# AU-Master-Thesis/magics

Hardware: AMD Instinct MI355X
Metric: GBP iterations/sec (whole node), N robots x K horizon (higher is better)
Workload: dtype f64

## Files before the change

include/mgx.h:

```cpp
#ifndef MGX_H
#define MGX_H

#include <stdint.h>

#ifdef __cplusplus
extern "C" {
#endif

#define MGX_DOFS 4

#define MGX_OK 0
#define MGX_ERR_INVALID (-1)
#define MGX_ERR_NO_DEVICE (-2)
#define MGX_ERR_HIP (-3)
#define MGX_ERR_STATE (-4)
#define MGX_ERR_NOMEM (-5)

#define MGX_FACTOR_DYNAMIC 1u
#define MGX_FACTOR_INTERROBOT 2u
#define MGX_FACTOR_OBSTACLE 4u
#define MGX_FACTOR_TRACKING 8u

#define MGX_STEP_INTERNAL 1u
#define MGX_STEP_EXTERNAL 2u
// ... 76 lines not shown
#define MGX_SWEEP_FORM_SHARDED 3
int mgx_last_sweep(mgx_world *w, int32_t *variant, int32_t *ir_mode, int32_t *form, int32_t *resident_capacity);
#define MGX_SEARCH_NONE -1
#define MGX_SEARCH_TWO_PASS_PAIRS 0
#define MGX_SEARCH_TWO_PASS_GRID 1
#define MGX_SEARCH_ROWS_PAIRS_4 2
#define MGX_SEARCH_ROWS_PAIRS_2 3
#define MGX_SEARCH_ROWS_GRID_16 4
#define MGX_SEARCH_ROWS_GRID_32 5
int mgx_last_search(mgx_world *w, int32_t *kernel, int32_t *row_cap, int32_t *n_launches, int32_t *n_changed, uint8_t *changed,
                    uint32_t capacity);

int mgx_flush(mgx_world *w);
int mgx_set_linger(mgx_world *w, int32_t microseconds );
int mgx_linger_stats(mgx_world *w, uint64_t *launches, uint64_t *posts, uint64_t *reruns, uint64_t *ended_by_device);
int mgx_set_resident_launches(mgx_world *w, int32_t enabled);
int mgx_is_thawing(mgx_world *w, int32_t *thawing);

#define MGX_HINT_NEXT_STARTS_EXTERNAL 1u
int mgx_sweep(mgx_world *w, int32_t robot, uint32_t external_phases, uint32_t internal_phases,
              uint32_t n_internal, uint32_t hints);

int mgx_internal_factor_iteration(mgx_world *w, int32_t robot);
int mgx_internal_variable_iteration(mgx_world *w, int32_t robot);
int mgx_external_factor_iteration(mgx_world *w, int32_t robot);
int mgx_external_variable_iteration(mgx_world *w, int32_t robot);

int mgx_change_prior(mgx_world *w, int32_t robot, uint32_t var_ix, const double mean[4]);
int mgx_change_priors(mgx_world *w, uint32_t n, const int32_t *robots, const uint32_t *var_ix,
                      const double *means);
// ... 300 lines not shown
```

include/mgx.hpp:

```cpp
#pragma once

#include <array>
#include <cstdint>
#include <limits>
#include <memory>
#include <optional>
#include <stdexcept>
#include <string>
#include <utility>
#include <vector>

#include "mgx.h"

namespace mgx {

struct Error : std::runtime_error {
    int code;
    Error(int c, const std::string &what) : std::runtime_error(what), code(c) {}
};
inline int check(int rc) {
    if (rc < 0) throw Error(rc, mgx_last_error());
    return rc;
}

// ... 115 lines not shown
        check(mgx_ir_connect(w_, owner.id(), other.id(), numbers.next_value));
        numbers.next_value += K_ - 1;
    }
    void tick(const std::vector<int32_t> &robots, const std::vector<double> &waypoints_xy, const std::vector<double> &time_scale,
              const std::vector<uint8_t> &what, double max_speed, double delta_t, const std::vector<uint8_t> &steps) {
        check(mgx_tick(w_, (uint32_t)robots.size(), robots.data(), waypoints_xy.data(), time_scale.data(), what.data(), max_speed,
                       delta_t, steps.data(), (uint32_t)steps.size()));
    }
    uint32_t last_launch_count() {
        uint32_t n = 0;
        check(mgx_last_launch_count(w_, &n));
        return n;
    }
    void flush() { check(mgx_flush(w_)); }
    void set_linger(int32_t microseconds) { check(mgx_set_linger(w_, microseconds)); }
    void change_factor_enabled(uint32_t kind_mask) { check(mgx_set_enabled(w_, kind_mask)); }
    void update_inter_robot_safety_distance_multiplier(double multiplier) { check(mgx_set_safety_multiplier(w_, multiplier)); }
    std::pair<uint32_t, uint32_t> update_topology(const std::vector<std::array<float, 3>> &translations, float comms_radius,
                                                  RobotNumberGenerator &numbers) {
        uint32_t stats[2] = {0, 0};
        check(mgx_update_topology(w_, translations[0].data(), comms_radius, MGX_NEIGHBOURS_AUTO, &numbers.next_value, stats));
        return {stats[0], stats[1]};
    }
    void iterate_gbp_v2(const std::vector<GbpScheduleAtIteration> &sched) {
        std::vector<uint8_t> steps(sched.size());
        for (size_t i = 0; i < sched.size(); i++) steps[i] = (uint8_t)((sched[i].internal ? MGX_STEP_INTERNAL : 0) | (sched[i].external ? MGX_STEP_EXTERNAL : 0));
        check(mgx_iterate(w_, steps.data(), (uint32_t)steps.size()));
    }
    struct Batch {
        mgx_world *w;
// ... 235 lines not shown
```

magics_amd/csrc/mgx_resident.h:

```cpp
#pragma once
#include <algorithm>
#include <cstddef>
#include <cstdint>
#include <vector>

namespace mgx {

#ifndef __HIPCC__
constexpr uint32_t PH_INT_FACTOR = 4u, PH_INT_VARIABLE = 8u;
constexpr int MAX_SEGS = 32;
#endif
static_assert((PH_INT_FACTOR | PH_INT_VARIABLE) == 12u && MAX_SEGS == 32, "the phases and the plan's size as mgx_dev.h has them");

struct Launch { uint32_t ext; int n_int; uint32_t hints; };
inline uint32_t int_phases(const Launch &l) { return l.n_int ? (PH_INT_FACTOR | PH_INT_VARIABLE) : 0; }

inline int fill_segments(const std::vector<Launch> &plan, size_t from, uint8_t *ext, uint8_t *n_int) {
    const int n = (int)std::min<size_t>((size_t)MAX_SEGS, plan.size() - std::min(from, plan.size()));
    for (int k = 0; k < MAX_SEGS; k++) {
        ext[k] = k < n && plan[from + (size_t)k].ext ? 1 : 0;
        n_int[k] = k < n ? (uint8_t)plan[from + (size_t)k].n_int : 0;
    }
    return n;
}
// ... 3 lines not shown
    unsigned long long flag_base = 0;
    Standing after_launch(int n) const { return {(cur + n) & 1, flag_base + (unsigned long long)n}; }
    Standing after_post(int n) const { return after_launch(n - 1); }
};

struct Backoff {
    int left = 0, len = 0;
    void declined(int segments) {
        len = std::min(std::max(2 * len, 64), 32768);
        left = len + segments;
    }
    void external_iteration() { if (left > 0) left--; }
    void went_ahead() { len = 0; }
};

struct RidingUpdates {
    const double *dev = nullptr;
    const double *host = nullptr;
    int slot = -1;
    double max_speed = 0.0, delta_t = 0.0;
    bool any() const { return dev || host; }
    bool postable() const { return !dev || host; }
};

}
```

magics_amd/csrc/mgx_world_abi.inc:

```
extern "C" {

const char *mgx_last_error(void) { return g_err.c_str(); }
int mgx_set_error_(int code, const char *text) {
    g_err = text ? text : "";
    return code;
}

int mgx_world_create(const mgx_params *params, mgx_world **out) {
    if (!params || !out) return fail(MGX_ERR_INVALID, "null argument");
    if (!(params->sigma_dynamics > 0) || !(params->sigma_interrobot > 0) || !(params->sigma_obstacle > 0) ||
        !(params->sigma_tracking > 0) || !(params->safety_multiplier > 0))
        return fail(MGX_ERR_INVALID, "sigmas and safety multiplier must be positive");
    if (!device_ok()) return fail(MGX_ERR_NO_DEVICE, "no usable HIP device (this library has no CPU path)");
    mgx_world *w = new (std::nothrow) mgx_world();
    if (!w) return fail(MGX_ERR_NOMEM, "out of memory");
    w->p = *params;
    w->trk_ever_on = (params->enable_mask & 8u) != 0;
    *out = w;
    return MGX_OK;
}

int mgx_world_destroy(mgx_world *w) {
    if (!w) return MGX_OK;
    w->batch.steps.clear();
// ... 32 lines not shown
    MGX_ENTER(w);
    if (!w) return fail(MGX_ERR_INVALID, "null world");
    return MGX_OK;
}
int mgx_set_linger(mgx_world *w, int32_t microseconds) {
    MGX_ENTER(w);
    if (!w) return fail(MGX_ERR_INVALID, "null world");
    w->res.set_linger(microseconds);
    return MGX_OK;
}
int mgx_linger_stats(mgx_world *w, uint64_t *launches, uint64_t *posts, uint64_t *reruns, uint64_t *ended_by_device) {
    MGX_ENTER_SCHEDULE(w);
    if (!w) return fail(MGX_ERR_INVALID, "null world");
    const ResidentLaunches::Linger &lg = w->res.linger;
    if (launches) *launches = lg.launches;
    if (posts) *posts = lg.posts + (lg.un.active ? 1u : 0u);
    if (reruns) *reruns = lg.reruns;
    if (ended_by_device) *ended_by_device = lg.ended_by_device;
    return MGX_OK;
}

int mgx_world_set_sdf(mgx_world *w, const uint8_t *rgb, uint32_t width, uint32_t height, double world_w, double world_h) {
    MGX_ENTER(w);
    if (!w || !rgb || !width || !height || !(world_w > 0) || !(world_h > 0)) return fail(MGX_ERR_INVALID, "bad sdf arguments");
    w->sdf_red.resize((size_t)width * height);
    for (size_t i = 0; i < w->sdf_red.size(); i++) w->sdf_red[i] = rgb[3 * i];
    w->sdf_w = width; w->sdf_h = height; w->world_w = world_w; w->world_h = world_h;
    w->dirty = w->relayout = true;
    return MGX_OK;
}

int mgx_world_set_environment(mgx_world *w, const mgx_env_desc *env) {
    MGX_ENTER(w);
// ... 346 lines not shown
```

magics_amd/csrc/mgx_world_launch.inc:

```
static int direct_exchange(mgx_world *w);
static int rccl_exchange(mgx_world *w);
static int sweep(mgx_world *w, int32_t robot, uint32_t ext_mask, uint32_t int_mask, int n_int, uint32_t hints = 0);
static void log_launch(mgx_world *w, int robot, uint32_t ext_mask, uint32_t int_mask, int n_int);

static void log_plan(mgx_world *w, const std::vector<Launch> &plan, size_t from = 0, size_t n = ~(size_t)0) {
    for (size_t k = from; k < plan.size() && k - from < n; k++) log_launch(w, -1, plan[k].ext, int_phases(plan[k]), plan[k].n_int);
}
static int run_segments(mgx_world *w, const std::vector<Launch> &plan, size_t from, const RidingUpdates &upd) {
    for (size_t k = from; k < plan.size(); k++) {
        const bool rides = k == from && upd.dev;
        if (rides) { w->d.upd = upd.dev; w->d.upd_max_speed = upd.max_speed; w->d.upd_delta_t = upd.delta_t; }
        int rc = sweep(w, -1, plan[k].ext, int_phases(plan[k]), plan[k].n_int, plan[k].hints);
        w->d.upd = nullptr;
        if (rides && upd.slot >= 0) {
            const hipError_t e = w->stage.release(upd.slot, w->stream);
            if (rc == MGX_OK && e != hipSuccess) rc = fail(MGX_ERR_HIP, "event record: %s", hipGetErrorString(e));
        }
        if (rc != MGX_OK) return rc;
    }
    return MGX_OK;
}
template <class F>
static int spin_until(F done) {
    const double t0 = StageTimer::now();
// ... 130 lines not shown
        if (w->thaw_kinds && (thawing || writes_snap)) HIP_TRY(launch_thaw_done(w->d, w->dev_of[(size_t)robot], 1, writes_snap ? 1 : 0, w->stream));
        log_launch(w, robot, 0, int_mask, n_int);
    }
    return MGX_OK;
}


struct ResidentKnobs {
    static long long positive(const char *name, long long dflt) { const char *e = getenv(name); const long long v = e ? atoll(e) : dflt; return v > 0 ? v : dflt; }
    static bool persistent() { static const bool v = [] { const char *e = getenv("MGX_PERSISTENT"); return !(e && e[0] == '0'); }(); return v; }
    static long long timeout_ticks() { static const long long v = positive("MGX_RESIDENT_TIMEOUT_MS", 2000) * 100000ll; return v; }
    static bool census() { static const bool v = [] { const char *e = getenv("MGX_RESIDENT_CENSUS"); return !(e && e[0] == '0'); }(); return v; }
    static long long census_ticks() { static const long long v = positive("MGX_RESIDENT_CENSUS_US", 200) * 100ll; return v; }
    static long long census_ticks_sharded() { static const long long v = positive("MGX_RESIDENT_CENSUS_SHARDED_US", 20000) * 100ll; return v; }
    static bool cooperative() { static const bool v = [] { const char *e = getenv("MGX_COOPERATIVE"); return e && e[0] == '1'; }(); return v; }
    static long long linger_ticks() {
        const char *off = getenv("MGX_LINGER"), *us = getenv("MGX_LINGER_US");
        const long long v = off && off[0] == '0' ? 0 : us ? atoll(us) : 300;
        return (v > 0 ? std::min<long long>(v, 1000000) : 0) * 100ll;
    }
};
static bool resident_enabled() { return ResidentKnobs::persistent(); }
static int ensure_resident_tables(mgx_world *w) {
    hipStream_t s = w->stream;
    const size_t R = (size_t)w->d.R_local;
    if (!w->res.sweep_abort_buf.p) {
        std::vector<unsigned long long> z(1, 0ull);
        HIP_TRY(w->res.sweep_abort_buf.upload(z, s));
        HIP_TRY(hipStreamSynchronize(s));
    }
// ... 79 lines not shown
enum ResidentFit { FITS, UNFIT_NOW, UNFIT_LDS, UNFIT_CAPACITY };
static ResidentFit resident_fits(mgx_world *w, bool sharded) {
    const DevWorld &d = w->d;
    if (!(d.ir_max_edges > 0 && !w->conns.empty() && !w->thaw_kinds && !w->ir_thaw_active && w->n_keyless == 0 && w->res.mode != ResidentLaunches::DECLINE))
        return UNFIT_NOW;
    if (sweep_lds_bytes(w->K, d.ir_max_edges, true) > sweep_resident_lds_max()) return UNFIT_LDS;
    return d.R_local + 1 > w->res.capacity_for(d, sharded) ? UNFIT_CAPACITY : FITS;
}

static int run_resident(mgx_world *w, const std::vector<Launch> &plan);
static long long linger_ticks(mgx_world *w) {
    ResidentLaunches::Linger &lg = w->res.linger;
    if (lg.ticks < 0) lg.ticks = ResidentKnobs::linger_ticks();
    return lg.ticks;
}
static double *linger_upd_slot(mgx_world *w, unsigned long long number) {
    ResidentLaunches::Linger &lg = w->res.linger;
    return reinterpret_cast<double *>(reinterpret_cast<char *>(lg.box()) + sizeof(LingerBox)) + (size_t)(number & 1ull) * lg.upd_stride;
}
static int ensure_linger_box(mgx_world *w) {
    ResidentLaunches::Linger &lg = w->res.linger;
    const size_t stride = ((size_t)4 * (size_t)std::max(w->d.R_local, 1) + 7) & ~(size_t)7;
    if (!lg.go.p) {
        std::vector<unsigned long long> z(1, 0ull);
        HIP_TRY(lg.go.upload(z, w->stream));
        HIP_TRY(hipStreamSynchronize(w->stream));
    }
    if (lg.box() && lg.upd_stride >= stride) return MGX_OK;
    const size_t grown = (stride + stride / 2 + 7) & ~(size_t)7;
    HIP_TRY(lg.box_mem.alloc(sizeof(LingerBox) + 2 * grown * sizeof(double)));
// ... 7 lines not shown
template <class F>
static int linger_wait(mgx_world *w, F pred, const char *what) {
    ResidentLaunches::Linger &lg = w->res.linger;
    const int r = spin_until([&] {
        if (pred()) return 1;
        const unsigned long long c = __atomic_load_n(&lg.box()->closed, __ATOMIC_ACQUIRE);
        return (c & 1ull) && (c >> 1) >= lg.seq0 ? 2 : 0;
    });
    if (r < 0) return fail(MGX_ERR_STATE, "lingering launch %llu: no answer from the device while waiting for %s (the stream does not advance)", lg.seq0, what);
    return r - 1;
}
static void linger_confirm(mgx_world *w) {
    ResidentLaunches::Linger &lg = w->res.linger;
    log_plan(w, lg.un.plan);
    lg.un.active = false;
    lg.posts++;
    lg.taken_in_launch++;
}
static int run_schedule(mgx_world *w, const std::vector<Launch> &plan, const RidingUpdates &upd, StageTimer *lap = nullptr) {
    const RidingUpdates outer = w->res.riding;
    w->res.riding = upd;
    const int resident = run_resident(w, plan);
    w->res.riding = outer;
    if (lap) lap->lap("resident launch enqueued");
    if (resident == 0) return run_segments(w, plan, 0, upd);
    const hipError_t e = upd.slot >= 0 ? w->stage.release(upd.slot, w->stream) : hipSuccess;
    if (resident < 0) return resident;
    return e == hipSuccess ? MGX_OK : fail(MGX_ERR_HIP, "event record: %s", hipGetErrorString(e));
}
static int linger_settle(mgx_world *w, bool nested = false) {
    ResidentLaunches::Linger &lg = w->res.linger;
    const uint32_t count_before = w->last_sweep_launches;
    const unsigned long long c = __atomic_load_n(&lg.box()->closed, __ATOMIC_ACQUIRE);
    lg.open = false;
    int rc = MGX_OK;
    if (lg.un.active && (c >> 1) >= lg.un.number) {
        linger_confirm(w);
    } else if (lg.un.active) {
        Submitted un = std::move(lg.un);
        lg.un = Submitted{};
        lg.reruns++;
        un.take_back(w);
        RidingUpdates upd;
        if (un.upd.any()) {
            const size_t bytes = 4 * (size_t)w->d.R_local * sizeof(double);
            void *hp = nullptr, *dp = nullptr;
            HIP_TRY(w->stage.acquire(bytes, &hp, &upd.slot));
            memcpy(hp, un.upd.host, bytes);
            HIP_TRY(hipHostGetDevicePointer(&dp, hp, 0));
            upd.dev = (const double *)dp;
            upd.host = (const double *)hp;
            upd.max_speed = un.upd.max_speed;
            upd.delta_t = un.upd.delta_t;
        }
        rc = run_schedule(w, un.plan, upd);
    }
    if (nested) w->last_sweep_launches = count_before;
    if (lg.taken_in_launch == 0) lg.useless++;
    else lg.useless = 0;
    return rc;
}
static int linger_close(mgx_world *w) {
    ResidentLaunches::Linger &lg = w->res.linger;
    if (!lg.open) return MGX_OK;
    const int rc = confirm_held(w);
    if (rc != MGX_OK || !lg.open) return rc;
    StageTimer clock("linger");
    __atomic_store_n(&lg.box()->close_req, lg.seq0, __ATOMIC_RELEASE);
    const int r = linger_wait(w, [] { return false; }, "the launch to end");
    if (r < 0) return r;
    clock.lap("closed");
    return linger_settle(w);
}
static bool linger_plan_fits(const std::vector<Launch> &plan) {
    if (plan.empty() || plan.size() > (size_t)MAX_SEGS || plan[0].ext) return false;
    for (const Launch &l : plan)
        if (l.n_int > 255) return false;
    return true;
}
static int linger_prepare_post(mgx_world *w, const std::vector<Launch> &plan) {
    ResidentLaunches &rl = w->res;
    ResidentLaunches::Linger &lg = rl.linger;
    if (!lg.open) return 0;
    {
        const uint32_t count_before = w->last_sweep_launches;
        const int rc = confirm_held(w);
        w->last_sweep_launches = count_before;
        if (rc != MGX_OK) return rc;
        if (!lg.open) return 0;
    }
    const bool fits = linger_plan_fits(plan) && !w->dirty && !w->conns_dirty && !w->flags_dirty && !w->thaw_kinds && !w->ir_thaw_active &&
                      w->n_keyless == 0 && rl.mode == ResidentLaunches::ON && (w->p.enable_mask & 2u) && rl.backoff.left == 0;
    if (!fits) {
        const int rc = linger_close(w);
        return rc != MGX_OK ? rc : 0;
    }
    int r = 0;
    if (lg.un.active) {
        const unsigned long long n = lg.un.number;
        r = linger_wait(w, [&] { return __atomic_load_n(&lg.box()->taken, __ATOMIC_ACQUIRE) >= n; }, "the last post to be taken");
        if (r == 0) linger_confirm(w);
    }
    if (r < 0) return r;
    if (r == 1) {
        lg.ended_by_device++;
        const int rc = linger_settle(w, true);
        return rc != MGX_OK ? rc : 0;
// ... 7 lines not shown
    LingerPlan &lp = lg.box()->plan[P & 1ull];
    lp.n = (uint32_t)plan.size();
    lp.has_upd = upd.any() ? 1u : 0u;
    uint8_t ext[MAX_SEGS], n_int[MAX_SEGS];
    fill_segments(plan, 0, ext, n_int);
    memcpy(lp.ext, ext, sizeof ext);
    memcpy(lp.n_int, n_int, sizeof n_int);
    lp.upd_max_speed = upd.max_speed;
    lp.upd_delta_t = upd.delta_t;
    lp.number = P;
    Submitted &un = lg.un;
    un.active = true;
    un.number = P;
    un.plan = plan;
    un.before = standing(w);
    un.upd = RidingUpdates{};
    if (upd.any()) {
        double *slot = linger_upd_slot(w, P);
        if (upd.host != slot) memcpy(slot, upd.host, 4 * (size_t)w->d.R_local * sizeof(double));
        un.upd.host = slot;
        un.upd.max_speed = upd.max_speed;
        un.upd.delta_t = upd.delta_t;
    }
    __atomic_store_n(&lg.box()->posted, P, __ATOMIC_RELEASE);
    stand_at(w, un.before.after_post((int)plan.size()));
    w->stale_kinds |= ~w->p.enable_mask & 15u;
    w->last_sweep_launches++;
    w->last_sweep = lg.ran;
    w->last_sweep_form = MGX_SWEEP_FORM_POSTED;
}
// ... 129 lines not shown
```

magics_amd/csrc/mgx_world_schedule.inc:

```
extern "C" {
static int submit_batch(mgx_world *w) {
    std::vector<uint8_t> st;
    st.swap(w->batch.steps);
    if (st.empty()) return MGX_OK;
    const int rc = iterate_now(w, st.data(), (uint32_t)st.size());
    w->batch.submissions++;
    w->batch.launches += w->last_sweep_launches;
    return rc;
}

int mgx_batch_begin(mgx_world *w) {
    if (!w) return fail(MGX_ERR_INVALID, "null world");
    if (w->batch.open) return fail(MGX_ERR_STATE, "a batch is open already");
    w->batch.open = true;
    w->batch.schedules = w->batch.submissions = w->batch.launches = 0;
    return MGX_OK;
}
int mgx_batch_end(mgx_world *w, uint32_t *n_schedules, uint32_t *n_launches) {
    if (!w) return fail(MGX_ERR_INVALID, "null world");
    if (!w->batch.open) return fail(MGX_ERR_STATE, "no batch is open");
    w->batch.open = false;
    const int rc = submit_batch(w);
    if (n_schedules) *n_schedules = w->batch.schedules;
    if (n_launches) *n_launches = w->batch.launches;
    return rc;
}

int mgx_iterate(mgx_world *w, const uint8_t *steps, uint32_t n) {
    if (!w || (!steps && n)) return fail(MGX_ERR_INVALID, "null argument");
    for (uint32_t i = 0; i < n; i++)
        if (steps[i] & ~(MGX_STEP_INTERNAL | MGX_STEP_EXTERNAL)) return fail(MGX_ERR_INVALID, "bad step %u", i);
    if (!w->batch.open) return iterate_now(w, steps, n);
    if (w->robots.empty()) return fail(MGX_ERR_STATE, "world has no robots");
    int rc0 = check_device_error(w);
    if (rc0 != MGX_OK) return rc0;
    mgx_world::Batch &b = w->batch;
    if (!b.steps.empty()) {
        std::vector<uint8_t> both(b.steps);
        both.insert(both.end(), steps, steps + n);
        if (plan_launches(both.data(), (uint32_t)both.size()).size() > (size_t)MAX_SEGS) {
            const int rc = submit_batch(w);
            if (rc != MGX_OK) return rc;
        }
    }
    b.steps.insert(b.steps.end(), steps, steps + n);
    b.schedules++;
    return MGX_OK;
}

static int iterate_now(mgx_world *w, const uint8_t *steps, uint32_t n) {
    const std::vector<Launch> plan = plan_launches(steps, n);
    const int rcc = confirm_held(w);
    if (rcc != MGX_OK) return rcc;
    w->last_sweep_launches = 0;
    w->last_sweep = SweepRan{};
    w->last_sweep_form = -1;
    w->res.schedule_issued();
    return run_schedule(w, plan, RidingUpdates{});
}

int mgx_internal_factor_iteration(mgx_world *w, int32_t robot) {
    MGX_ENTER(w);
    return w ? sweep(w, robot, 0, PH_INT_FACTOR, 1) : fail(MGX_ERR_INVALID, "null world");
}
int mgx_internal_variable_iteration(mgx_world *w, int32_t robot) {
    MGX_ENTER(w);
// ... 533 lines not shown
```

magics_amd/csrc/mgx_world_types.h:

```cpp
#pragma once
#include <hip/hip_runtime.h>

#include <algorithm>
#include <cmath>
#include <cstdarg>
#include <cstdio>
#include <cstdlib>
#include <dlfcn.h>
#include <cstring>
#include <map>
#include <memory>
#include <string>
#include <utility>
#include <vector>

#include "../../include/mgx.h"
#include "gbp_math.h"
#include "mgx_dev.h"
#include "mgx_grid.h"
#include "mgx_search.h"
#include "mgx_plan_pool.h"
#include "mgx_resident.h"

namespace mgx {
// ... 378 lines not shown
    void release() { if (p) (void)hipHostFree(p); p = nullptr; }
    hipError_t alloc(size_t bytes) {
        release();
        const hipError_t e = hipHostMalloc(&p, bytes, hipHostMallocMapped);
        if (e == hipSuccess) memset(p, 0, bytes);
        return e;
    }
};

struct Submitted {
    bool active = false;
    unsigned long long number = 0;
    std::vector<Launch> plan;
    Standing before;
    bool partial = false;
    RidingUpdates upd;
    void take_back(mgx_world *w);
};

struct ResidentLaunches {
    DevBuf<unsigned long long> sweep_flag_buf, sweep_abort_buf, census_buf, decision_buf;
    DevBuf<unsigned char> xrec_buf;
    MappedBlock decision_mem;
    unsigned long long *decision_host() const { return (unsigned long long *)decision_mem.p; }
    DevBuf<int32_t> peer_ptr_dev, peer_ptr_dev_b;
    size_t peer_idx_off = 0;
    std::vector<int32_t> peer_fill;
    bool peers_valid = false;
    unsigned long long flag_base = 0;
    unsigned long long launch_seq = 0;
// ... 12 lines not shown
        long long ticks = -1;
        MappedBlock box_mem;
        LingerBox *box() const { return (LingerBox *)box_mem.p; }
        size_t upd_stride = 0;
        DevBuf<unsigned long long> go;
        DevBuf<unsigned char> dev;
        size_t dev_stride = 0;
        bool open = false, hold = false;
        unsigned long long seq0 = 0;
        SweepRan ran;
        uint32_t taken_in_launch = 0;
        int useless = 0;
        uint32_t streak = 0;
        Submitted un;
        uint64_t launches = 0, posts = 0, reruns = 0, ended_by_device = 0;
    } linger;
    void arrays_rebuilt() {
        peers_valid = false;
        sweep_flag_buf.n = 0;
        flag_base = 0;
        cap = cap_sharded = -1;
    }
    void robots_appended() {
        peers_valid = false;
        sweep_flag_buf.n = 0;
        flag_base = 0;
    }
    void lds_footprint_changed() { cap = cap_sharded = -1; }
    void peers_rebuilt(bool built, size_t R, DevWorld &d) {
        if (built) {
// ... 70 lines not shown
    DevBuf<IrEdgeRec> ir_rec_b;
    DevBuf<int32_t> in_ptr_dev, in_ptr_dev_b, in_mid_dev;
    DevBuf<IrSlotRec> slot_recs, slot_recs_b;
    std::vector<int32_t> dev_in_ptr;
    DevBuf<int32_t> trk_record, path_ptr, iter_factor, ir_var_ptr, ir_var_mid;
    DevBuf<uint32_t> epoch0, epoch1;
    DevBuf<float> trk_last_pos, path_xy;
    DevBuf<uint8_t> ir_gate, antenna, idle, sdf;
    DevBuf<double> radius_dev;
    StageRing stage;
    unsigned long long *sweep_err_host = nullptr;
    struct Batch {
        bool open = false;
        std::vector<uint8_t> steps;
        uint32_t schedules = 0, submissions = 0, launches = 0;
    } batch;
    ResidentLaunches res;
    int sticky_rc = 0;
    struct ConnHot {
        int32_t owner, other, node_first, node_last;
        uint64_t first_number;
        int32_t dev_q;
        uint8_t has_fresh;
    };
    std::vector<ConnHot> conn_hot;
    ConnIndex cidx;
    struct Cum { std::vector<uint64_t> nIv, nEv, nEf, on_ir; } cum;
    bool conns_unsettled = false;
    std::vector<uint8_t> scratch_dead;
    std::vector<int32_t> scratch_dead_list;
// ... 239 lines not shown
```

magics_amd/hostlib.py:

```python
import ctypes as C
import os

_HERE = os.path.dirname(os.path.abspath(__file__))
LIB_PATH = os.path.join(_HERE, "lib", "libmgx.so")
FMA_LIB_PATH = os.path.join(_HERE, "lib", "libmgx_fma.so")

SCHEDULE_CENTERED = 0
SCHEDULE_SOON_AS_POSSIBLE = 1
SCHEDULE_LATE_AS_POSSIBLE = 2
SCHEDULE_INTERLEAVE_EVENLY = 3
SCHEDULE_HALF_BEGINNING_HALF_END = 4

STEP_INTERNAL = 1
STEP_EXTERNAL = 2
NEIGHBOURS_AUTO, NEIGHBOURS_PAIRS, NEIGHBOURS_GRID = 0, 1, 2
GLOBAL_PATH_RESET_TRACKING, GLOBAL_PATH_ROUTE, GLOBAL_PATH_ACTIVATE = 1, 2, 4
RESIDENT_NONE, RESIDENT_RAN, RESIDENT_DECLINED = 0, 1, 2
SEARCH_NONE, SEARCH_TWO_PASS_PAIRS, SEARCH_TWO_PASS_GRID, SEARCH_ROWS_PAIRS_4, SEARCH_ROWS_PAIRS_2, SEARCH_ROWS_GRID_16, SEARCH_ROWS_GRID_32 = -1, 0, 1, 2, 3, 4, 5
HALO_PUSH, HALO_WAIT = 1, 2
HINT_NEXT_STARTS_EXTERNAL = 1

c_double_p = C.POINTER(C.c_double)


# ... 170 lines not shown
    "mgx_collisions_update": (C.c_int, [_V, C.c_void_p]),
    "mgx_collisions_read": (C.c_int, [_V, C.c_uint64, C.c_void_p, C.c_uint64, C.POINTER(C.c_uint64), C.POINTER(C.c_uint64), C.c_void_p]),
    "mgx_collisions_clear": (C.c_int, [_V]),
    "mgx_tracks_enable": (C.c_int, [_V, C.c_int32, C.c_uint64, C.c_uint64, C.c_uint64, C.c_uint64]),
    "mgx_tracks_set_clock": (C.c_int, [_V, C.c_uint64]),
    "mgx_tracks_update": (C.c_int, [_V, C.c_void_p, C.c_void_p, C.c_uint64]),
    "mgx_tracks_take": (C.c_int, [_V, C.c_void_p, C.c_uint64, C.POINTER(C.c_uint64), C.POINTER(C.c_uint64), C.POINTER(C.c_uint64), C.c_void_p]),
    "mgx_tracks_clear": (C.c_int, [_V]),
    "mgx_num_robots": (C.c_int, [_V, C.POINTER(C.c_uint32), C.POINTER(C.c_uint32)]),
    "mgx_last_launch_count": (C.c_int, [_V, C.POINTER(C.c_uint32)]),
    "mgx_last_sweep": (C.c_int, [_V, C.POINTER(C.c_int32), C.POINTER(C.c_int32), C.POINTER(C.c_int32), C.POINTER(C.c_int32)]),
    "mgx_last_search": (C.c_int, [_V, C.POINTER(C.c_int32), C.POINTER(C.c_int32), C.POINTER(C.c_int32), C.POINTER(C.c_int32), _V, C.c_uint32]),
    "mgx_flush": (C.c_int, [_V]),
    "mgx_set_linger": (C.c_int, [_V, C.c_int32]),
    "mgx_linger_stats": (C.c_int, [_V, C.POINTER(C.c_uint64), C.POINTER(C.c_uint64), C.POINTER(C.c_uint64), C.POINTER(C.c_uint64)]),
    "mgx_set_resident_launches": (C.c_int, [_V, C.c_int32]),
    "mgx_is_thawing": (C.c_int, [_V, C.POINTER(C.c_int32)]),
    "mgx_halo_words": (C.c_uint32, [C.c_uint32]),
    "mgx_halo_plan": (C.c_int, [_V, C.c_uint32, C.POINTER(C.c_int32), C.c_uint32, C.POINTER(C.c_int32)]),
    "mgx_halo_plan_from_connections": (C.c_int, [_V, C.POINTER(C.c_int32), C.c_uint32, C.c_int32, C.c_uint32, C.POINTER(C.c_uint32),
                                                 C.POINTER(C.c_uint32)]),
    "mgx_shard_partition": (C.c_int, [c_double_p, C.c_uint32, C.c_uint32, C.POINTER(C.c_int32)]),
    "mgx_shard_plan_create": (C.c_int, [C.POINTER(C.c_int32), C.c_uint32, C.POINTER(C.c_int32), C.POINTER(C.c_int32), C.c_uint32, C.c_int32,
                                        C.c_uint32, C.POINTER(_V)]),
    "mgx_shard_plan_destroy": (None, [_V]),
    "mgx_shard_plan_counts": (C.c_int, [_V] + [C.POINTER(C.c_uint32)] * 5),
    "mgx_shard_plan_get": (C.c_int, [_V, C.POINTER(C.c_int32), C.POINTER(C.c_int32), C.POINTER(C.c_uint32), C.POINTER(C.c_uint32),
                                     C.POINTER(C.c_int32), C.POINTER(C.c_uint32), C.POINTER(C.c_int32)]),
    "mgx_halo_pack": (C.c_int, [_V, _V]),
    "mgx_halo_unpack": (C.c_int, [_V, _V]),
# ... 243 lines not shown
```

magics_amd/world.py:

```python
import ctypes as C

import numpy as np

from . import hostlib
from .hostlib import Params, RobotDesc, c_double_p
from .hostlib import check as _check


def _dp(a):
    return a.ctypes.data_as(c_double_p)


def _f64(a, shape=None):
    a = np.ascontiguousarray(a, dtype=np.float64)
    if shape is not None and a.shape != shape:
        raise ValueError(f"expected shape {shape}, got {a.shape}")
    return a


def make_params(p):
    return Params(
        float(p["sigma_dynamics"]), float(p["sigma_interrobot"]), float(p["sigma_obstacle"]),
        float(p["sigma_tracking"]), float(p["safety_multiplier"]),
        float(p.get("tracking_switch_padding", 1.0)), float(p.get("tracking_attraction_distance", 2.0)),
# ... 32 lines not shown
        self._chk(self._L.mgx_set_stream(self._w, C.c_void_p(int(stream))))
        self.stream_handle = int(stream)

    def synchronize(self):
        self._chk(self._L.mgx_synchronize(self._w))

    def flush(self):
        self._chk(self._L.mgx_flush(self._w))

    def set_linger(self, microseconds):
        self._chk(self._L.mgx_set_linger(self._w, -1 if microseconds is None else int(microseconds)))

    def linger_stats(self):
        v = [C.c_uint64() for _ in range(4)]
        self._chk(self._L.mgx_linger_stats(self._w, *[C.byref(x) for x in v]))
        return tuple(int(x.value) for x in v)

    def set_sdf(self, rgb, world_w, world_h):
        rgb = np.ascontiguousarray(rgb, dtype=np.uint8)
        if rgb.ndim != 3 or rgb.shape[2] != 3:
            raise ValueError("rgb must be HxWx3 u8")
        h, w, _ = rgb.shape
        self._chk(self._L.mgx_world_set_sdf(self._w, rgb.ctypes.data, w, h, float(world_w), float(world_h)))

    def set_environment(self, env):
        from .environment import _Desc
        d = _Desc(env)
        self._chk(self._L.mgx_world_set_environment(self._w, C.byref(d.desc)))

    def add_robot(self, mean0, prior_diag, dt, radius, path=None, order_key=None, ghost=False):
# ... 678 lines not shown
```

rust/magics-hip/src/lib.rs:

```rust
pub mod sys;

use std::ffi::CStr;
use std::sync::Arc;

#[derive(Debug)]
pub struct MgxError(pub i32, pub String);

fn check(rc: i32) -> Result<(), MgxError> {
    if rc >= 0 {
        return Ok(());
    }
    let msg = unsafe { CStr::from_ptr(sys::mgx_last_error()) }.to_string_lossy().into_owned();
    Err(MgxError(rc, msg))
}

pub struct World {
    raw: *mut sys::mgx_world,
}
unsafe impl Send for World {}
unsafe impl Sync for World {}

impl World {
    pub fn new(params: sys::mgx_params) -> Result<Arc<Self>, MgxError> {
        let mut raw = std::ptr::null_mut();
// ... 82 lines not shown
        r?;
        e?;
        Ok((schedules, launches))
    }
    pub fn last_launch_count(&self) -> Result<u32, MgxError> {
        let mut n = 0u32;
        check(unsafe { sys::mgx_last_launch_count(self.raw, &mut n) })?;
        Ok(n)
    }
    pub fn flush(&self) -> Result<(), MgxError> {
        check(unsafe { sys::mgx_flush(self.raw) })
    }
    pub fn set_linger(&self, microseconds: i32) -> Result<(), MgxError> {
        check(unsafe { sys::mgx_set_linger(self.raw, microseconds) })
    }
    pub fn resident_stats(&self) -> Result<(u64, u64, u32), MgxError> {
        let (mut launches, mut declined, mut backoff) = (0u64, 0u64, 0u32);
        check(unsafe { sys::mgx_resident_stats(self.raw, &mut launches, &mut declined, &mut backoff) })?;
        Ok((launches, declined, backoff))
    }
    #[allow(clippy::too_many_arguments)]
    pub fn tick(&self, robots: &[i32], waypoints_xy: &[[f64; 2]], time_scale: &[f64], what: &[u8],
                max_speed: f64, delta_t: f64, steps: &[u8]) -> Result<(), MgxError> {
        assert!(robots.len() == waypoints_xy.len() && robots.len() == time_scale.len() && robots.len() == what.len());
        check(unsafe {
            sys::mgx_tick(self.raw, robots.len() as u32, robots.as_ptr(), waypoints_xy.as_ptr().cast(), time_scale.as_ptr(),
                          what.as_ptr(), max_speed, delta_t, steps.as_ptr(), steps.len() as u32)
        })
    }
    pub fn change_priors(&self, robots: &[i32], vars: &[u32], means: &[[f64; 4]]) -> Result<(), MgxError> {
// ... 143 lines not shown
```

rust/magics-hip/src/sys.rs:

```rust
#![allow(non_camel_case_types)]
use std::os::raw::{c_char, c_int, c_void};

#[repr(C)]
pub struct mgx_world { _private: [u8; 0] }

#[repr(C)]
#[derive(Clone, Copy)]
pub struct mgx_params {
    pub sigma_dynamics: f64,
    pub sigma_interrobot: f64,
    pub sigma_obstacle: f64,
    pub sigma_tracking: f64,
    pub safety_multiplier: f64,
    pub tracking_switch_padding: f64,
    pub tracking_attraction_distance: f64,
    pub enable_mask: u32,
    pub reserved: u32,
}

#[repr(C)]
pub struct mgx_robot_desc {
    pub k: u32,
    pub n_path: u32,
    pub mean0: *const f64,
// ... 201 lines not shown
    pub fn mgx_set_antenna(w: *mut mgx_world, robot: i32, active: i32) -> c_int;
    pub fn mgx_set_idle(w: *mut mgx_world, robot: i32, idle: i32) -> c_int;
    pub fn mgx_set_antennas(w: *mut mgx_world, n: u32, robots: *const i32, active: *const u8) -> c_int;
    pub fn mgx_neighbours(w: *mut mgx_world, positions_xyz: *const f32, radius: f32, method: u32, row_ptr: *mut i32, neighbours_out: *mut i32, capacity: u64, needed: *mut u64) -> c_int;
    pub fn mgx_update_topology(w: *mut mgx_world, positions_xyz: *const f32, radius: f32, method: u32, robot_number_next: *mut u64, stats: *mut u32) -> c_int;
    pub fn mgx_connections(w: *mut mgx_world, robot: i32, others: *mut i32, capacity: u32, n: *mut u32) -> c_int;
    pub fn mgx_iterate(w: *mut mgx_world, steps: *const u8, n: u32) -> c_int;
    pub fn mgx_batch_begin(w: *mut mgx_world) -> c_int;
    pub fn mgx_batch_end(w: *mut mgx_world, n_schedules: *mut u32, n_launches: *mut u32) -> c_int;
    pub fn mgx_last_launch_count(w: *mut mgx_world, n_launches: *mut u32) -> c_int;
    pub fn mgx_last_sweep(w: *mut mgx_world, variant: *mut i32, ir_mode: *mut i32, form: *mut i32, resident_capacity: *mut i32) -> c_int;
    pub fn mgx_last_search(w: *mut mgx_world, kernel: *mut i32, row_cap: *mut i32, n_launches: *mut i32, n_changed: *mut i32, changed: *mut u8, capacity: u32) -> c_int;
    pub fn mgx_flush(w: *mut mgx_world) -> c_int;
    pub fn mgx_set_linger(w: *mut mgx_world, microseconds: i32) -> c_int;
    pub fn mgx_linger_stats(w: *mut mgx_world, launches: *mut u64, posts: *mut u64, reruns: *mut u64, ended_by_device: *mut u64) -> c_int;
    pub fn mgx_set_resident_launches(w: *mut mgx_world, enabled: i32) -> c_int;
    pub fn mgx_is_thawing(w: *mut mgx_world, thawing: *mut i32) -> c_int;
    pub fn mgx_sweep(w: *mut mgx_world, robot: i32, external_phases: u32, internal_phases: u32, n_internal: u32, hints: u32) -> c_int;
    pub fn mgx_internal_factor_iteration(w: *mut mgx_world, robot: i32) -> c_int;
    pub fn mgx_internal_variable_iteration(w: *mut mgx_world, robot: i32) -> c_int;
    pub fn mgx_external_factor_iteration(w: *mut mgx_world, robot: i32) -> c_int;
    pub fn mgx_external_variable_iteration(w: *mut mgx_world, robot: i32) -> c_int;
    pub fn mgx_change_prior(w: *mut mgx_world, robot: i32, var_ix: u32, mean: *const f64) -> c_int;
    pub fn mgx_change_priors(w: *mut mgx_world, n: u32, robots: *const i32, var_ix: *const u32, means: *const f64) -> c_int;
    pub fn mgx_reset_variables(w: *mut mgx_world, robot: i32, means: *const f64, n_means: u32, first_last_sigma: f64, inbetween_sigma: f64) -> c_int;
    pub fn mgx_reset_tracking_factors(w: *mut mgx_world, robot: i32) -> c_int;
    pub fn mgx_set_tracking_path(w: *mut mgx_world, robot: i32, path_xy: *const f32, n_path: u32) -> c_int;
    pub fn mgx_apply_global_paths(w: *mut mgx_world, n: u32, robots: *const i32, path_ptr: *const u32, path_xy: *const f32, means: *const f64, first_last_sigma: f64, inbetween_sigma: f64, flags: u32) -> c_int;
    pub fn mgx_layout_stats(w: *mut mgx_world, n_layouts: *mut u64, n_pulls: *mut u64) -> c_int;
    pub fn mgx_world_reserve(w: *mut mgx_world, robots: u32) -> c_int;
// ... 102 lines not shown
```

Before: 130,300.

## Merge consecutive iterate calls into one lingering post when device is behind

Adds a post-merge mode, AUTO by default, that holds an incoming mgx_iterate schedule on the host when a lingering resident launch already has untaken posts outstanding. The held steps are later submitted together with following schedules as one combined plan. The goal is fewer host-to-device posts and less per-post handshake overhead. In exchange it adds host-side deferral logic and merged-plan bookkeeping, and linger_close now waits for the last post to be taken; deferred work could add latency or change ordering around flushes.

```diff
diff --git a/include/mgx.h b/include/mgx.h
--- a/include/mgx.h
+++ b/include/mgx.h
@@ -114,6 +114,8 @@
 int mgx_flush(mgx_world *w);
 int mgx_set_linger(mgx_world *w, int32_t microseconds );
 int mgx_linger_stats(mgx_world *w, uint64_t *launches, uint64_t *posts, uint64_t *reruns, uint64_t *ended_by_device);
+int mgx_set_post_merge(mgx_world *w, int32_t mode );
+int mgx_post_merge_stats(mgx_world *w, uint64_t *plans_posted, uint64_t *schedules_in_them, uint64_t *largest);
 int mgx_set_resident_launches(mgx_world *w, int32_t enabled);
 int mgx_is_thawing(mgx_world *w, int32_t *thawing);
 
diff --git a/include/mgx.hpp b/include/mgx.hpp
--- a/include/mgx.hpp
+++ b/include/mgx.hpp
@@ -153,6 +153,7 @@
     }
     void flush() { check(mgx_flush(w_)); }
     void set_linger(int32_t microseconds) { check(mgx_set_linger(w_, microseconds)); }
+    void set_post_merge(int32_t mode) { check(mgx_set_post_merge(w_, mode)); }
     void change_factor_enabled(uint32_t kind_mask) { check(mgx_set_enabled(w_, kind_mask)); }
     void update_inter_robot_safety_distance_multiplier(double multiplier) { check(mgx_set_safety_multiplier(w_, multiplier)); }
     std::pair<uint32_t, uint32_t> update_topology(const std::vector<std::array<float, 3>> &translations, float comms_radius,
diff --git a/magics_amd/csrc/mgx_resident.h b/magics_amd/csrc/mgx_resident.h
--- a/magics_amd/csrc/mgx_resident.h
+++ b/magics_amd/csrc/mgx_resident.h
@@ -41,6 +41,25 @@
     void went_ahead() { len = 0; }
 };
 
+inline bool linger_plan_fits(const std::vector<Launch> &plan) {
+    if (plan.empty() || plan.size() > (size_t)MAX_SEGS || plan[0].ext) return false;
+    for (const Launch &l : plan)
+        if (l.n_int > 255) return false;
+    return true;
+}
+
+enum PostMergeMode : int32_t { POST_MERGE_OFF = 0, POST_MERGE_AUTO = 1, POST_MERGE_ALWAYS = 2 };
+enum class PostMerge { SUBMIT, DEFER, SUBMIT_RECORDED };
+inline PostMerge post_merge_decide(int32_t mode, bool launch_open, unsigned outstanding, bool taken, bool qualifies, bool held,
+                                   const std::vector<Launch> &fresh, const std::vector<Launch> &merged) {
+    if (fresh.empty()) return held ? PostMerge::SUBMIT_RECORDED : PostMerge::SUBMIT;
+    const bool post_untaken = outstanding > 2u && !taken;
+    const bool joins = linger_plan_fits(merged) && (mode == POST_MERGE_ALWAYS || linger_plan_fits(fresh));
+    if (held && !joins) return PostMerge::SUBMIT_RECORDED;
+    const bool record = mode != POST_MERGE_OFF && launch_open && qualifies && joins && (mode == POST_MERGE_ALWAYS || post_untaken);
+    return record ? PostMerge::DEFER : PostMerge::SUBMIT;
+}
+
 struct RidingUpdates {
     const double *dev = nullptr;
     const double *host = nullptr;
diff --git a/magics_amd/csrc/mgx_world_abi.inc b/magics_amd/csrc/mgx_world_abi.inc
--- a/magics_amd/csrc/mgx_world_abi.inc
+++ b/magics_amd/csrc/mgx_world_abi.inc
@@ -70,9 +70,26 @@
     if (!w) return fail(MGX_ERR_INVALID, "null world");
     const ResidentLaunches::Linger &lg = w->res.linger;
     if (launches) *launches = lg.launches;
-    if (posts) *posts = lg.posts + (lg.un.active ? 1u : 0u);
+    if (posts) *posts = lg.posts + (lg.un.active ? lg.un.schedules : 0u);
     if (reruns) *reruns = lg.reruns;
     if (ended_by_device) *ended_by_device = lg.ended_by_device;
+    return MGX_OK;
+}
+
+int mgx_set_post_merge(mgx_world *w, int32_t mode) {
+    MGX_ENTER_SCHEDULE(w);
+    if (!w) return fail(MGX_ERR_INVALID, "null world");
+    if (mode > POST_MERGE_ALWAYS) return fail(MGX_ERR_INVALID, "bad post-merge mode %d", mode);
+    w->res.linger.merge_mode = mode < 0 ? -1 : mode;
+    return MGX_OK;
+}
+int mgx_post_merge_stats(mgx_world *w, uint64_t *plans_posted, uint64_t *schedules_in_them, uint64_t *largest) {
+    MGX_ENTER_SCHEDULE(w);
+    if (!w) return fail(MGX_ERR_INVALID, "null world");
+    const ResidentLaunches::Linger &lg = w->res.linger;
+    if (plans_posted) *plans_posted = lg.plans_posted;
+    if (schedules_in_them) *schedules_in_them = lg.schedules_in_plans;
+    if (largest) *largest = lg.largest_plan;
     return MGX_OK;
 }
 
diff --git a/magics_amd/csrc/mgx_world_launch.inc b/magics_amd/csrc/mgx_world_launch.inc
--- a/magics_amd/csrc/mgx_world_launch.inc
+++ b/magics_amd/csrc/mgx_world_launch.inc
@@ -168,6 +168,10 @@
     static long long census_ticks() { static const long long v = positive("MGX_RESIDENT_CENSUS_US", 200) * 100ll; return v; }
     static long long census_ticks_sharded() { static const long long v = positive("MGX_RESIDENT_CENSUS_SHARDED_US", 20000) * 100ll; return v; }
     static bool cooperative() { static const bool v = [] { const char *e = getenv("MGX_COOPERATIVE"); return e && e[0] == '1'; }(); return v; }
+    static int32_t post_merge() {
+        const char *e = getenv("MGX_POST_MERGE");
+        return e && e[0] >= '0' && e[0] <= '2' && !e[1] ? e[0] - '0' : POST_MERGE_AUTO;
+    }
     static long long linger_ticks() {
         const char *off = getenv("MGX_LINGER"), *us = getenv("MGX_LINGER_US");
         const long long v = off && off[0] == '0' ? 0 : us ? atoll(us) : 300;
@@ -277,6 +281,11 @@
     if (lg.ticks < 0) lg.ticks = ResidentKnobs::linger_ticks();
     return lg.ticks;
 }
+static int32_t post_merge_mode(mgx_world *w) {
+    ResidentLaunches::Linger &lg = w->res.linger;
+    if (lg.merge_mode < 0) lg.merge_mode = ResidentKnobs::post_merge();
+    return lg.merge_mode;
+}
 static double *linger_upd_slot(mgx_world *w, unsigned long long number) {
     ResidentLaunches::Linger &lg = w->res.linger;
     return reinterpret_cast<double *>(reinterpret_cast<char *>(lg.box()) + sizeof(LingerBox)) + (size_t)(number & 1ull) * lg.upd_stride;
@@ -314,7 +323,7 @@
     ResidentLaunches::Linger &lg = w->res.linger;
     log_plan(w, lg.un.plan);
     lg.un.active = false;
-    lg.posts++;
+    lg.posts += lg.un.schedules;
     lg.taken_in_launch++;
 }
 static int run_schedule(mgx_world *w, const std::vector<Launch> &plan, const RidingUpdates &upd, StageTimer *lap = nullptr) {
@@ -339,7 +348,7 @@
     } else if (lg.un.active) {
         Submitted un = std::move(lg.un);
         lg.un = Submitted{};
-        lg.reruns++;
+        lg.reruns += un.schedules;
         un.take_back(w);
         RidingUpdates upd;
         if (un.upd.any()) {
@@ -366,22 +375,28 @@
     const int rc = confirm_held(w);
     if (rc != MGX_OK || !lg.open) return rc;
     StageTimer clock("linger");
+    if (lg.un.active) {
+        const unsigned long long n = lg.un.number;
+        const int r0 = linger_wait(w, [&] { return __atomic_load_n(&lg.box()->taken, __ATOMIC_ACQUIRE) >= n; }, "the last post to be taken");
+        if (r0 < 0) return r0;
+        if (r0 == 1) return linger_settle(w);
+    }
     __atomic_store_n(&lg.box()->close_req, lg.seq0, __ATOMIC_RELEASE);
     const int r = linger_wait(w, [] { return false; }, "the launch to end");
     if (r < 0) return r;
     clock.lap("closed");
     return linger_settle(w);
 }
-static bool linger_plan_fits(const std::vector<Launch> &plan) {
-    if (plan.empty() || plan.size() > (size_t)MAX_SEGS || plan[0].ext) return false;
-    for (const Launch &l : plan)
-        if (l.n_int > 255) return false;
-    return true;
+static bool linger_world_qualifies(const mgx_world *w) {
+    const ResidentLaunches &rl = w->res;
+    return !w->dirty && !w->conns_dirty && !w->flags_dirty && !w->thaw_kinds && !w->ir_thaw_active && w->n_keyless == 0 &&
+           rl.mode == ResidentLaunches::ON && (w->p.enable_mask & 2u) && rl.backoff.left == 0;
 }
 static int linger_prepare_post(mgx_world *w, const std::vector<Launch> &plan) {
     ResidentLaunches &rl = w->res;
     ResidentLaunches::Linger &lg = rl.linger;
     if (!lg.open) return 0;
+    if (const int rce = check_device_error(w)) return rce;
     {
         const uint32_t count_before = w->last_sweep_launches;
         const int rc = confirm_held(w);
@@ -389,8 +404,7 @@
         if (rc != MGX_OK) return rc;
         if (!lg.open) return 0;
     }
-    const bool fits = linger_plan_fits(plan) && !w->dirty && !w->conns_dirty && !w->flags_dirty && !w->thaw_kinds && !w->ir_thaw_active &&
-                      w->n_keyless == 0 && rl.mode == ResidentLaunches::ON && (w->p.enable_mask & 2u) && rl.backoff.left == 0;
+    const bool fits = linger_plan_fits(plan) && linger_world_qualifies(w);
     if (!fits) {
         const int rc = linger_close(w);
         return rc != MGX_OK ? rc : 0;
@@ -428,6 +442,10 @@
     un.number = P;
     un.plan = plan;
     un.before = standing(w);
+    un.schedules = std::max(lg.coming, 1u);
+    lg.plans_posted++;
+    lg.schedules_in_plans += un.schedules;
+    lg.largest_plan = std::max<uint64_t>(lg.largest_plan, un.schedules);
     un.upd = RidingUpdates{};
     if (upd.any()) {
         double *slot = linger_upd_slot(w, P);
diff --git a/magics_amd/csrc/mgx_world_schedule.inc b/magics_amd/csrc/mgx_world_schedule.inc
--- a/magics_amd/csrc/mgx_world_schedule.inc
+++ b/magics_amd/csrc/mgx_world_schedule.inc
@@ -2,14 +2,68 @@
 static int submit_batch(mgx_world *w) {
     std::vector<uint8_t> st;
     st.swap(w->batch.steps);
+    const uint32_t merged = w->batch.implicit;
+    w->batch.implicit = 0;
     if (st.empty()) return MGX_OK;
+    ResidentLaunches::Linger &lg = w->res.linger;
+    if (merged > 1) lg.streak += merged - 1;
+    lg.coming = std::max(merged, 1u);
     const int rc = iterate_now(w, st.data(), (uint32_t)st.size());
+    lg.coming = 1;
     w->batch.submissions++;
     w->batch.launches += w->last_sweep_launches;
     return rc;
 }
 
+static int iterate_plan(mgx_world *w, const std::vector<Launch> &plan);
+static bool linger_open_now(mgx_world *w, int *rc) {
+    ResidentLaunches::Linger &lg = w->res.linger;
+    *rc = MGX_OK;
+    if (!lg.open) return false;
+    const uint32_t count_before = w->last_sweep_launches;
+    *rc = confirm_held(w);
+    w->last_sweep_launches = count_before;
+    if (*rc != MGX_OK || !lg.open) return false;
+    const unsigned long long c = __atomic_load_n(&lg.box()->closed, __ATOMIC_ACQUIRE);
+    return !((c & 1ull) && (c >> 1) >= lg.seq0);
+}
+static int iterate_merging(mgx_world *w, const uint8_t *steps, uint32_t n) {
+    mgx_world::Batch &b = w->batch;
+    ResidentLaunches::Linger &lg = w->res.linger;
+    const int32_t mode = post_merge_mode(w);
+    if (mode == POST_MERGE_OFF && b.steps.empty()) return iterate_now(w, steps, n);
+    if (w->robots.empty()) return fail(MGX_ERR_STATE, "world has no robots");
+    int rc = check_device_error(w);
+    if (rc != MGX_OK) return rc;
+    const std::vector<Launch> fresh = plan_launches(steps, n);
+    for (int round = 0; round < 2; round++) {
+        const bool held = !b.steps.empty();
+        std::vector<Launch> merged_plan;
+        if (held) {
+            std::vector<uint8_t> both(b.steps);
+            both.insert(both.end(), steps, steps + n);
+            merged_plan = plan_launches(both.data(), (uint32_t)both.size());
+        }
+        const std::vector<Launch> &merged = held ? merged_plan : fresh;
+        const bool open = linger_open_now(w, &rc);
+        if (rc != MGX_OK) return rc;
+        const unsigned outstanding = open && lg.un.active ? (unsigned)std::min<unsigned long long>(lg.un.number - lg.seq0, 1000ull) : 0u;
+        const bool taken = outstanding && __atomic_load_n(&lg.box()->taken, __ATOMIC_ACQUIRE) >= lg.un.number;
+        const PostMerge what = post_merge_decide(mode, open, outstanding, taken, linger_world_qualifies(w), held, fresh, merged);
+        if (what == PostMerge::SUBMIT_RECORDED) {
+            if ((rc = submit_batch(w)) != MGX_OK) return rc;
+            continue;
+        }
+        if (what == PostMerge::SUBMIT && !held) return iterate_plan(w, fresh);
+        b.steps.insert(b.steps.end(), steps, steps + n);
+        b.implicit++;
+        return what == PostMerge::DEFER ? MGX_OK : submit_batch(w);
+    }
+    return fail(MGX_ERR_STATE, "internal: a schedule was neither recorded nor submitted");
+}
+
 int mgx_batch_begin(mgx_world *w) {
+    MGX_ENTER_SCHEDULE(w);
     if (!w) return fail(MGX_ERR_INVALID, "null world");
     if (w->batch.open) return fail(MGX_ERR_STATE, "a batch is open already");
     w->batch.open = true;
@@ -30,7 +84,10 @@
     if (!w || (!steps && n)) return fail(MGX_ERR_INVALID, "null argument");
     for (uint32_t i = 0; i < n; i++)
         if (steps[i] & ~(MGX_STEP_INTERNAL | MGX_STEP_EXTERNAL)) return fail(MGX_ERR_INVALID, "bad step %u", i);
-    if (!w->batch.open) return iterate_now(w, steps, n);
+    if (!w->batch.open) {
+        if (!w->res.linger.open && w->batch.steps.empty()) return iterate_now(w, steps, n);
+        return iterate_merging(w, steps, n);
+    }
     if (w->robots.empty()) return fail(MGX_ERR_STATE, "world has no robots");
     int rc0 = check_device_error(w);
     if (rc0 != MGX_OK) return rc0;
@@ -48,8 +105,8 @@
     return MGX_OK;
 }
 
-static int iterate_now(mgx_world *w, const uint8_t *steps, uint32_t n) {
-    const std::vector<Launch> plan = plan_launches(steps, n);
+static int iterate_now(mgx_world *w, const uint8_t *steps, uint32_t n) { return iterate_plan(w, plan_launches(steps, n)); }
+static int iterate_plan(mgx_world *w, const std::vector<Launch> &plan) {
     const int rcc = confirm_held(w);
     if (rcc != MGX_OK) return rcc;
     w->last_sweep_launches = 0;
diff --git a/magics_amd/csrc/mgx_world_types.h b/magics_amd/csrc/mgx_world_types.h
--- a/magics_amd/csrc/mgx_world_types.h
+++ b/magics_amd/csrc/mgx_world_types.h
@@ -416,6 +416,7 @@
     std::vector<Launch> plan;
     Standing before;
     bool partial = false;
+    uint32_t schedules = 1;
     RidingUpdates upd;
     void take_back(mgx_world *w);
 };
@@ -458,6 +459,9 @@
         uint32_t streak = 0;
         Submitted un;
         uint64_t launches = 0, posts = 0, reruns = 0, ended_by_device = 0;
+        int32_t merge_mode = -1;
+        uint32_t coming = 1;
+        uint64_t plans_posted = 0, schedules_in_plans = 0, largest_plan = 0;
     } linger;
     void arrays_rebuilt() {
         peers_valid = false;
@@ -558,6 +562,7 @@
         bool open = false;
         std::vector<uint8_t> steps;
         uint32_t schedules = 0, submissions = 0, launches = 0;
+        uint32_t implicit = 0;
     } batch;
     ResidentLaunches res;
     int sticky_rc = 0;
diff --git a/magics_amd/hostlib.py b/magics_amd/hostlib.py
--- a/magics_amd/hostlib.py
+++ b/magics_amd/hostlib.py
@@ -208,6 +208,8 @@
     "mgx_flush": (C.c_int, [_V]),
     "mgx_set_linger": (C.c_int, [_V, C.c_int32]),
     "mgx_linger_stats": (C.c_int, [_V, C.POINTER(C.c_uint64), C.POINTER(C.c_uint64), C.POINTER(C.c_uint64), C.POINTER(C.c_uint64)]),
+    "mgx_set_post_merge": (C.c_int, [_V, C.c_int32]),
+    "mgx_post_merge_stats": (C.c_int, [_V, C.POINTER(C.c_uint64), C.POINTER(C.c_uint64), C.POINTER(C.c_uint64)]),
     "mgx_set_resident_launches": (C.c_int, [_V, C.c_int32]),
     "mgx_is_thawing": (C.c_int, [_V, C.POINTER(C.c_int32)]),
     "mgx_halo_words": (C.c_uint32, [C.c_uint32]),
diff --git a/magics_amd/world.py b/magics_amd/world.py
--- a/magics_amd/world.py
+++ b/magics_amd/world.py
@@ -70,6 +70,14 @@
     def linger_stats(self):
         v = [C.c_uint64() for _ in range(4)]
         self._chk(self._L.mgx_linger_stats(self._w, *[C.byref(x) for x in v]))
+        return tuple(int(x.value) for x in v)
+
+    def set_post_merge(self, mode):
+        self._chk(self._L.mgx_set_post_merge(self._w, -1 if mode is None else int(mode)))
+
+    def post_merge_stats(self):
+        v = [C.c_uint64() for _ in range(3)]
+        self._chk(self._L.mgx_post_merge_stats(self._w, *[C.byref(x) for x in v]))
         return tuple(int(x.value) for x in v)
 
     def set_sdf(self, rgb, world_w, world_h):
diff --git a/rust/magics-hip/src/lib.rs b/rust/magics-hip/src/lib.rs
--- a/rust/magics-hip/src/lib.rs
+++ b/rust/magics-hip/src/lib.rs
@@ -120,6 +120,9 @@
     pub fn set_linger(&self, microseconds: i32) -> Result<(), MgxError> {
         check(unsafe { sys::mgx_set_linger(self.raw, microseconds) })
     }
+    pub fn set_post_merge(&self, mode: i32) -> Result<(), MgxError> {
+        check(unsafe { sys::mgx_set_post_merge(self.raw, mode) })
+    }
     pub fn resident_stats(&self) -> Result<(u64, u64, u32), MgxError> {
         let (mut launches, mut declined, mut backoff) = (0u64, 0u64, 0u32);
         check(unsafe { sys::mgx_resident_stats(self.raw, &mut launches, &mut declined, &mut backoff) })?;
diff --git a/rust/magics-hip/src/sys.rs b/rust/magics-hip/src/sys.rs
--- a/rust/magics-hip/src/sys.rs
+++ b/rust/magics-hip/src/sys.rs
@@ -239,6 +239,8 @@
     pub fn mgx_flush(w: *mut mgx_world) -> c_int;
     pub fn mgx_set_linger(w: *mut mgx_world, microseconds: i32) -> c_int;
     pub fn mgx_linger_stats(w: *mut mgx_world, launches: *mut u64, posts: *mut u64, reruns: *mut u64, ended_by_device: *mut u64) -> c_int;
+    pub fn mgx_set_post_merge(w: *mut mgx_world, mode: i32) -> c_int;
+    pub fn mgx_post_merge_stats(w: *mut mgx_world, plans_posted: *mut u64, schedules_in_them: *mut u64, largest: *mut u64) -> c_int;
     pub fn mgx_set_resident_launches(w: *mut mgx_world, enabled: i32) -> c_int;
     pub fn mgx_is_thawing(w: *mut mgx_world, thawing: *mut i32) -> c_int;
     pub fn mgx_sweep(w: *mut mgx_world, robot: i32, external_phases: u32, internal_phases: u32, n_internal: u32, hints: u32) -> c_int;
```

Result: faster. 137,200, median of 6 (+5.3%).
